# bacpop/sparrowhawk

Measured on AMD Instinct MI355X. Metric: Gbases/s assembled, k=31 150bp reads, higher is better.
Workload: dtype u64

## Files before the change

sparrowhawk_amd/csrc/ctl_words.h:

```cpp
#pragma once
#include <stddef.h>
#include <stdint.h>

namespace shk {

static constexpr int CTL_WORDS = 32;

struct CountWords {
    union { unsigned long long row_cursor;
            unsigned long long g_instances; };
    union { unsigned long long instances;
            unsigned long long g_overflow; };
    uint32_t part_too_large, bucket_splits;
    uint32_t n_handed_over, tally;
    unsigned long long bucket_list_len;
    unsigned long long spare5[4];
    unsigned long long bloom_keys;
    unsigned long long spare10;
    unsigned long long probe_work;
    unsigned long long dedupe_work;
    unsigned long long spare13;
    uint32_t groups_out, group_tally;
    unsigned long long spare15[7];
    unsigned long long er_cursor;
    unsigned long long er_broken;
    unsigned long long spare24[8];
};
struct P1Words {
    uint32_t spare, seg_too_long;
    unsigned long long max_fill;
};
struct CountMail {
    CountWords w;
    unsigned long long hist[500];
    P1Words p1;
};
static constexpr int COUNT_MAIL_WORDS = (int)(sizeof(CountMail) / 8);
static_assert(sizeof(CountMail) == (CTL_WORDS + 500 + 2) * 8 && offsetof(CountMail, hist) == CTL_WORDS * 8 && offsetof(CountMail, p1) == (CTL_WORDS + 500) * 8,
              "CountMail: words, histogram, pass 1's flags, contiguous");
static inline unsigned tally_tried(uint32_t t) { return t & 0xFFFFu; }
static inline unsigned tally_over(uint32_t t) { return t >> 16; }
static inline unsigned long long er_rows(unsigned long long cursor) { return cursor >> 32; }

struct GraphWords {
    unsigned long long spare0;
    unsigned long long table_flag;
    unsigned long long slots_used;
    unsigned long long n_cand, n_tips;
    union { unsigned long long tips_removed;
            unsigned long long n_splitters; };
    union { unsigned long long bubbles_removed;
            unsigned long long n_chains; };
    unsigned long long n_ring_splitters;
    uint32_t collapse_flag, n_spl_wanted;
    unsigned long long n_alive;
    unsigned long long n_walked;
    unsigned long long n_fork_cand;
    unsigned long long spare12;
    union { unsigned long long xq_count;
            unsigned long long halflink_flags; };
    unsigned long long writer_flag;
    unsigned long long spare15;
    unsigned long long r0_tips_removed, r0_bubbles_removed;
    unsigned long long plan_state, plan_bytes, plan_emitted;
    unsigned long long spare21[11];
};

#define SHK_CTL_AT(S, m, slot, half) static_assert(offsetof(S, m) == (slot) * 8 + (half) * 4, #S "::" #m " moved")
static_assert(sizeof(CountWords) == CTL_WORDS * 8 && sizeof(GraphWords) == CTL_WORDS * 8, "32 control words");
SHK_CTL_AT(CountWords, row_cursor, 0, 0);     SHK_CTL_AT(CountWords, g_instances, 0, 0);
SHK_CTL_AT(CountWords, instances, 1, 0);      SHK_CTL_AT(CountWords, g_overflow, 1, 0);
SHK_CTL_AT(CountWords, part_too_large, 2, 0); SHK_CTL_AT(CountWords, bucket_splits, 2, 1);
SHK_CTL_AT(CountWords, n_handed_over, 3, 0);  SHK_CTL_AT(CountWords, tally, 3, 1);
SHK_CTL_AT(CountWords, bucket_list_len, 4, 0);
SHK_CTL_AT(CountWords, bloom_keys, 9, 0);
SHK_CTL_AT(CountWords, probe_work, 11, 0);    SHK_CTL_AT(CountWords, dedupe_work, 12, 0);
SHK_CTL_AT(CountWords, groups_out, 14, 0);    SHK_CTL_AT(CountWords, group_tally, 14, 1);
SHK_CTL_AT(CountWords, er_cursor, 22, 0);     SHK_CTL_AT(CountWords, er_broken, 23, 0);
SHK_CTL_AT(GraphWords, spare0, 0, 0);         SHK_CTL_AT(GraphWords, table_flag, 1, 0);
SHK_CTL_AT(GraphWords, slots_used, 2, 0);     SHK_CTL_AT(GraphWords, n_cand, 3, 0);
SHK_CTL_AT(GraphWords, n_tips, 4, 0);
SHK_CTL_AT(GraphWords, tips_removed, 5, 0);   SHK_CTL_AT(GraphWords, n_splitters, 5, 0);
SHK_CTL_AT(GraphWords, bubbles_removed, 6, 0); SHK_CTL_AT(GraphWords, n_chains, 6, 0);
SHK_CTL_AT(GraphWords, n_ring_splitters, 7, 0);
SHK_CTL_AT(GraphWords, collapse_flag, 8, 0);  SHK_CTL_AT(GraphWords, n_spl_wanted, 8, 1);
SHK_CTL_AT(GraphWords, n_alive, 9, 0);        SHK_CTL_AT(GraphWords, n_walked, 10, 0);
SHK_CTL_AT(GraphWords, n_fork_cand, 11, 0);
SHK_CTL_AT(GraphWords, xq_count, 13, 0);      SHK_CTL_AT(GraphWords, halflink_flags, 13, 0);
SHK_CTL_AT(GraphWords, writer_flag, 14, 0);
SHK_CTL_AT(GraphWords, r0_tips_removed, 16, 0); SHK_CTL_AT(GraphWords, r0_bubbles_removed, 17, 0);
SHK_CTL_AT(GraphWords, plan_state, 18, 0);    SHK_CTL_AT(GraphWords, plan_bytes, 19, 0);
SHK_CTL_AT(GraphWords, plan_emitted, 20, 0);
#undef SHK_CTL_AT

}
```

sparrowhawk_amd/csrc/graph_part.h:

```cpp
#pragma once

struct MinScan {
    Nt32State first, last;
    uint32_t h_first, h_last;
    uint32_t min_wo_first;
    uint32_t min_wo_last;
    __device__ __forceinline__ uint32_t min_all() const { return min(min_wo_first, h_first); }
};

template <int W> __device__ __forceinline__ uint32_t km_base(const Kmer<W> &x, int k, int j) {
    return km_bits2<W>(x, 2 * (k - 1 - j));
}

template <int W> __device__ __forceinline__ MinScan km_min_scan(const Kmer<W> &x, int k, int gm) {
    MinScan r;
    Nt32State nt{0, 0};
    for (int j = 0; j < gm; j++) nt32_init_step(nt, km_base<W>(x, k, j), (unsigned)j);
    r.first = nt; r.h_first = nt32_canonical(nt);
    r.min_wo_first = 0xFFFFFFFFu; r.min_wo_last = r.h_first;
    const int w = k - gm + 1;
    uint32_t h = r.h_first;
    for (int q = 1; q < w; q++) {
        nt32_roll(nt, km_base<W>(x, k, q - 1), km_base<W>(x, k, q + gm - 1), (unsigned)gm);
        h = nt32_canonical(nt);
// ... 518 lines not shown
    const uint32_t *cnt;
    uint8_t *adj;
    GraphTable gt;
    const uint32_t *nb;
    int k;
    uint32_t n;
    uint32_t xref = 0;
    __device__ __forceinline__ uint32_t outmask(uint32_t v) const { return outmask_of(adj[v >> 1], v & 1); }
    __device__ __forceinline__ uint32_t outdeg(uint32_t v) const { return __popc(outmask(v)); }
    __device__ __forceinline__ uint32_t indeg(uint32_t v) const { return __popc(outmask(v ^ 1)); }
    __device__ __forceinline__ Kmer<W> seq(uint32_t v) const {
        Kmer<W> x = keys.load(v >> 1);
        return (v & 1) ? km_revcomp<W>(x, k) : x;
    }
    __device__ __forceinline__ uint32_t follow(uint32_t v, uint32_t b) const {
        Kmer<W> s = seq(v);
        km_push_back<W>(s, b, k);
        int o; Kmer<W> c = km_canonical<W>(s, k, o);
        uint32_t idx = gt_lookup<W>(gt, keys, c, k);
        return idx == NIL ? NIL : idx * 2 + (uint32_t)o;
    }
    __device__ __forceinline__ uint32_t only_out(uint32_t v) const {
        const uint32_t c = nb[v];
        if (c < NB_MULTI) return c;
        return follow(v, (uint32_t)__ffs((int)outmask(v)) - 1);
    }
};

struct TipRec { uint32_t start, junction, len, next; unsigned long long sum; };

template <int W>
__global__ __launch_bounds__(256) void k_tip_candidates(Graph<W> g, const uint8_t *__restrict__ alive,
                                                        uint32_t *__restrict__ cand,
                                                        unsigned int *__restrict__ n_cand,
                                                        uint2 *__restrict__ init_tip_head ,
                                                        uint8_t *__restrict__ init_mark ) {
    const int lane = threadIdx.x & 63;
    const uint32_t stride = gridDim.x * blockDim.x;
    const uint32_t n_round = (g.n + stride - 1) / stride * stride;
    for (uint32_t i = blockIdx.x * blockDim.x + threadIdx.x; i < n_round; i += stride) {
        uint32_t a = 0; bool al = false;
        if (i < g.n) {
            a = g.adj[i]; al = alive[i] != 0;
            if (init_tip_head) { uint2 nil; nil.x = NIL; nil.y = NIL; init_tip_head[i] = nil; init_mark[i] = 0; }
        }
#pragma unroll
        for (uint32_t o = 0; o < 2; o++) {
            const bool p = al && __popc(outmask_of(a, o ^ 1u)) == 0 && __popc(outmask_of(a, o)) == 1;
            const unsigned long long m = __ballot(p);
            if (!m) continue;
            unsigned int base = 0;
            if (lane == 0) base = atomicAdd(n_cand, (unsigned int)__popcll(m));
            base = __shfl(base, 0);
            if (p) cand[base + __popcll(m & ((1ull << lane) - 1ull))] = 2u * i + o;
        }
    }
}

template <int W>
__global__ __launch_bounds__(256) void k_tip_walk(Graph<W> g, const uint32_t *__restrict__ cand,
                                                  const unsigned int *__restrict__ n_cand_p, TipRec *__restrict__ tips,
                                                  unsigned int *__restrict__ n_tips,
                                                  uint32_t *__restrict__ tip_head) {
    const uint32_t T_TIP = 2u * (uint32_t)g.k;
    const uint32_t n_cand = *n_cand_p;
    for (uint32_t c = blockIdx.x * blockDim.x + threadIdx.x; c < n_cand; c += gridDim.x * blockDim.x) {
        const uint32_t v = cand[c];
        uint32_t cur = v, len = 1, J = NIL;
        unsigned long long sum = g.cnt[v >> 1];
        uint32_t a_cur = g.adj[cur >> 1], nb_cur = g.nb[cur];
        for (;;) {
            const uint32_t om = outmask_of(a_cur, cur & 1u);
            if (__popc(om) != 1) break;
            const uint32_t n = nb_cur < NB_MULTI ? nb_cur : g.follow(cur, (uint32_t)__ffs((int)om) - 1u);
            if (n == NIL) break;
            const uint32_t a_n = g.adj[n >> 1], nb_n = g.nb[n], c_n = g.cnt[n >> 1];
            if (__popc(outmask_of(a_n, (n & 1u) ^ 1u)) >= 2) { J = n; break; }
            len++; sum += c_n; cur = n; a_cur = a_n; nb_cur = nb_n;
            if (len > T_TIP) break;
        }
        if (J == NIL || len > T_TIP) continue;
        const uint32_t t = atomicAdd(n_tips, 1u);
        TipRec r; r.start = v; r.junction = J; r.len = len; r.sum = sum;
        r.next = atomicExch(&tip_head[J], t);
        tips[t] = r;
    }
}
// ... 42 lines not shown
}

__global__ __launch_bounds__(256) void k_tip_reset_heads(const TipRec *__restrict__ tips, const unsigned int *__restrict__ n_tips_p,
                                                         uint32_t *__restrict__ tip_head) {
    const uint32_t n_tips = *n_tips_p;
    for (uint32_t a = blockIdx.x * blockDim.x + threadIdx.x; a < n_tips; a += gridDim.x * blockDim.x)
        tip_head[tips[a].junction] = NIL;
}

template <int W>
__global__ __launch_bounds__(256) void k_fork_candidates(Graph<W> g, const uint8_t *__restrict__ alive,
                                                         uint32_t *__restrict__ cand,
                                                         unsigned int *__restrict__ n_cand) {
    const int lane = threadIdx.x & 63;
    const uint32_t stride = gridDim.x * blockDim.x;
    const uint32_t n_round = (g.n + stride - 1) / stride * stride;
    for (uint32_t i = blockIdx.x * blockDim.x + threadIdx.x; i < n_round; i += stride) {
        uint32_t a = 0; bool al = false;
        if (i < g.n) { a = g.adj[i]; al = alive[i] != 0; }
#pragma unroll
        for (uint32_t o = 0; o < 2; o++) {
            const bool p = al && __popc(outmask_of(a, o)) >= 2;
            const unsigned long long m = __ballot(p);
            if (!m) continue;
            unsigned int base = 0;
            if (lane == 0) base = atomicAdd(n_cand, (unsigned int)__popcll(m));
            base = __shfl(base, 0);
            if (p) cand[base + __popcll(m & ((1ull << lane) - 1ull))] = 2u * i + o;
        }
    }
}

template <int W>
__global__ __launch_bounds__(256) void k_bubble(Graph<W> g, const uint32_t *__restrict__ cand,
                                                const unsigned int *__restrict__ n_cand_p, uint8_t *__restrict__ mark) {
    const uint32_t T_BUB = 2u * (uint32_t)g.k;
    const uint32_t n_cand = *n_cand_p;
    for (uint32_t c = blockIdx.x * blockDim.x + threadIdx.x; c < n_cand; c += gridDim.x * blockDim.x) {
        const uint32_t S = cand[c];
        const uint32_t om = g.outmask(S);
        uint32_t first[4], end[4], len[4];
        unsigned long long sum[4];
        bool ok[4];
#pragma unroll
        for (uint32_t b = 0; b < 4; b++) {
            ok[b] = false; first[b] = NIL; end[b] = NIL; len[b] = 0; sum[b] = 0;
            if (!((om >> b) & 1u)) continue;
            const uint32_t bn = g.follow(S, b);
            if (bn == NIL || g.indeg(bn) != 1) continue;
            first[b] = bn;
            uint32_t cur = bn, l = 1;
            unsigned long long s = g.cnt[bn >> 1];
            for (;;) {
                if (g.outdeg(cur) != 1) break;
                const uint32_t n = g.only_out(cur);
                if (n == NIL) break;
                if (g.indeg(n) >= 2) { end[b] = n; ok[b] = true; break; }
                if (l + 1 > T_BUB) break;
                l++; s += g.cnt[n >> 1]; cur = n;
            }
            len[b] = l; sum[b] = s;
        }
#pragma unroll
        for (uint32_t a = 0; a < 4; a++) {
            if (!ok[a]) continue;
            const uint32_t E = end[a];
            {
                const Kmer<W> ks = g.keys.load(S >> 1), ke = g.keys.load(E >> 1);
                bool le;
                if (km_less<W>(ks, ke)) le = true;
                else if (km_less<W>(ke, ks)) le = false;
                else le = (S & 1u) <= ((E ^ 1u) & 1u);
                if (!le) continue;
            }
            uint32_t grp = 0; bool best = true;
            const Kmer<W> fa = g.keys.load(first[a] >> 1);
#pragma unroll
            for (uint32_t b = 0; b < 4; b++) {
                if (!ok[b] || end[b] != E) continue;
                grp++;
                if (b == a) continue;
                const unsigned long long l = sum[b] * len[a], r = sum[a] * len[b];
                bool better;
                if (l != r) better = l > r;
                else if (len[b] != len[a]) better = len[b] < len[a];
                else better = km_less<W>(g.keys.load(first[b] >> 1), fa);
                if (better) best = false;
            }
            if (grp >= 2 && !best) {
                uint32_t cur = first[a];
                for (uint32_t i = 0; i < len[a]; i++) {
                    mark[cur >> 1] = 1;
                    if (i + 1 < len[a]) cur = g.only_out(cur);
                }
            }
        }
    }
}

__global__ __launch_bounds__(256) void k_collect_marked(uint32_t n, uint8_t *__restrict__ mark,
                                                        uint8_t *__restrict__ alive,
                                                        uint32_t *__restrict__ removed,
                                                        unsigned int *__restrict__ n_removed) {
    const int lane = threadIdx.x & 63;
    const uint32_t stride = gridDim.x * blockDim.x;
    const uint32_t n_round = (n + stride - 1) / stride * stride;
    for (uint32_t i = blockIdx.x * blockDim.x + threadIdx.x; i < n_round; i += stride) {
        bool p = false;
        if (i < n && mark[i]) { mark[i] = 0; if (alive[i]) { alive[i] = 0; p = true; } }
        const unsigned long long m = __ballot(p);
        if (!m) continue;
        unsigned int base = 0;
        if (lane == 0) base = atomicAdd(n_removed, (unsigned int)__popcll(m));
        base = __shfl(base, 0);
        if (p) removed[base + __popcll(m & ((1ull << lane) - 1ull))] = i;
    }
}

__device__ __forceinline__ void adj_clear_bit(uint8_t *adj, uint32_t idx, uint32_t bit) {
    uint32_t *wptr = (uint32_t *)adj + (idx >> 2);
    atomicAnd(wptr, ~((1u << bit) << (8 * (idx & 3u))));
}

template <int W>
__global__ __launch_bounds__(256) void k_apply_removed(Graph<W> g, const uint32_t *__restrict__ removed,
                                                       const unsigned int *__restrict__ n_removed_p) {
    const uint32_t n_removed = *n_removed_p;
    for (uint32_t t = blockIdx.x * blockDim.x + threadIdx.x; t < n_removed; t += gridDim.x * blockDim.x) {
        const uint32_t r = removed[t];
        const uint32_t a = g.adj[r];
// ... 22 lines not shown
```

sparrowhawk_amd/csrc/pipeline.hip:

```cpp
#include <hip/hip_runtime.h>
#include <hipcub/hipcub.hpp>
#include <thread>
#include <stdint.h>
#include <stdio.h>
#include <stdlib.h>
#include <string.h>
#include <algorithm>
#include <atomic>
#include <chrono>
#include <map>
#include <memory>
#include <mutex>
#include <string>
#include <vector>

#include "ctl_words.h"
#include "device_mem.h"
#include "end_keys.h"
#include "kmer.h"
#include "pipeline.h"
#include "shard_comm.h"
#include "shard_plan.h"
#include "unitig_graph.h"
#include "unitig_graph_gpu.h"
// ... 1135 lines not shown
                            getenv("SHK_GP_ROWS") == nullptr && env_u64("SHK_GRAPH_RANGES", 1) != 0;
        er_ok_ = false;
        gp_ = 64;
        const uint64_t gp_rows_target = env_u64("SHK_GP_ROWS", 640);
        const uint64_t n_for_gp = sh_active_ ? n_solid_global_ : n;
        while (gp_ < GP_MAX && (uint64_t)gp_ * gp_rows_target < n_for_gp) gp_ <<= 1;
        if (ranges) gp_ = er_groups_;
        gt_slots_ = 4 * n + 8ull * gp_;
        if (int rc = gt_.alloc(gt_slots_, err)) return rc;
        if (int rc = gt_occ_.alloc(gt_slots_ / 8 + 8, err)) return rc;
        gt_scan_.release();
        if (!ranges && n && n <= (64ull << 20) && env_u64("SHK_KEEP_SCAN", 1)) if (int rc = gt_scan_.alloc(3 * n, err)) return rc;
        DevBuf<uint32_t> gp_of, gp_cnt, gp_roff, gp_rows, gp_n;
        if (ranges) {
            gt_off_.swap(er_off_); gt_msk_.swap(er_msk_); gp_roff.swap(er_start_); gp_n.swap(er_cnt_);
            er_off_.release(); er_msk_.release(); er_start_.release(); er_cnt_.release();
        } else {
            if (int rc = gt_off_.alloc(gp_, err)) return rc;
            if (int rc = gt_msk_.alloc(gp_, err)) return rc;
            if (int rc = gp_of.alloc(n, err)) return rc;
            if (int rc = gp_roff.alloc(gp_ + 1, err)) return rc;
            if (int rc = gp_rows.alloc(n, err)) return rc;
        }
        if (int rc = gp_cnt.alloc(gp_, err)) return rc;
        DevBuf<unsigned long long> queries;
        if (int rc = queries.alloc(8 * n + 8, err)) return rc;
        if (int rc = adj_.alloc((n + 8) & ~3ull, err)) return rc;
        if (keep_stages_) if (int rc = adj0_.alloc(n, err)) return rc;
        if (int rc = nb_.alloc(2 * n + 2, err)) return rc;
        if (int rc = alive_.alloc(n, err)) return rc;
        if (int rc = row_starts_.alloc(((n + 63) / 64) * 2 + 2, err)) return rc;
        if (ranges) HIPCHK(fill2_async(row_starts_.p, row_starts_.bytes, 0u, ctl_.p, sizeof(GraphWords), 0u, stream_));
        else HIPCHK(fill2_async(gp_cnt.p, (size_t)gp_ * 4, 0u, ctl_.p, sizeof(GraphWords), 0u, stream_));
        if (n || sh_active_) {
            Graph<W> g = graph_view();
            const uint32_t lowmask = std::min<uint32_t>(gp_, 256u) - 1u;
            if (ranges) {
                EvTimer t(stream_, stage_timers_);
                t.stop_later("graph_table_kernel", pending_timers_);
                EvTimer t2(stream_, stage_timers_);
                const GpRows gr{gp_roff.p, gp_n.p, nullptr};
                const uint32_t lds_slots = (uint32_t)std::min<uint64_t>(env_u64("SHK_GRAPH_LDS_SLOTS", ADJ_LDS_SLOTS_RANGES), ADJ_LDS_SLOTS_RANGES);
                hipLaunchKernelGGL((k_graph_local<W, ADJ_LDS_SLOTS_RANGES, ADJ_THREADS_RANGES>), dim3(gp_), dim3(ADJ_THREADS_RANGES), 0, stream_,
                                   g.keys, k_, g.gt, gr, adj_.p, nb_.p, queries.p, gp_cnt.p, (uint32_t *)ctl(&GraphWords::table_flag), lds_slots,
                                   alive_.p, row_starts_.p, lowmask);
                hipLaunchKernelGGL(k_graph_remote<W>, dim3(gp_), dim3(256), 0, stream_, g.keys, k_, g.gt, gr, queries.p,
                                   gp_cnt.p, adj_.p, nb_.p);
                HIPCHK(hipGetLastError());
                t2.stop_later("adjacency_kernel", pending_timers_);
                times_.add("graph_partitions_from_counting_x1", 1.0);
            } else {
                EvTimer t(stream_, stage_timers_);
                hipLaunchKernelGGL(k_gp_count<W>, dim3(grid_for(n)), dim3(256), 0, stream_, g.keys, (uint32_t)n, k_, g.gt,
                                   gp_of.p, gp_cnt.p);
                hipLaunchKernelGGL(k_gp_scan, dim3(1), dim3(1024), 0, stream_, gp_cnt.p, gp_, gt_off_.p, gt_msk_.p, gp_roff.p,
                                   ctl(&GraphWords::slots_used));
                hipLaunchKernelGGL(k_gp_rows, dim3(grid_for(n)), dim3(256), 0, stream_, gp_of.p, (uint32_t)n, gp_roff.p, gp_cnt.p,
                                   gp_rows.p);
                HIPCHK(hipGetLastError());
                if (n && (regroup_env == 1 || (regroup_env == 2 && rows_scattered_))) {
                    DevBuf<uint64_t> nk[W]; DevBuf<uint32_t> nc, ngp;
                    for (int j = 0; j < W; j++) if (int rc = nk[j].alloc(n, err)) return rc;
                    if (int rc = nc.alloc(n, err)) return rc;
                    if (int rc = ngp.alloc(n, err)) return rc;
                    KeyArr<W> out_keys; for (int j = 0; j < W; j++) out_keys.w[j] = nk[j].p;
                    hipLaunchKernelGGL(k_regroup_rows<W>, dim3(grid_for(n)), dim3(256), 0, stream_, g.keys, scnt_.p, gp_of.p, gp_rows.p, (uint32_t)n,
// ... 60 lines not shown
        unsigned long long h = 0;
        HIPCHK(hipMemcpyAsync(&h, ctl(m), ctl_span(m), hipMemcpyDeviceToHost, stream_));
        WAIT_STREAM();
        v = (unsigned int)h;
        return 0;
    }

    int apply_marks(Graph<W> &g, DevBuf<uint8_t> &mark, DevBuf<uint32_t> &removed, unsigned long long GraphWords::*m, std::string &err) {
        const uint32_t n = (uint32_t)n_solid_;
        hipLaunchKernelGGL(k_collect_marked, dim3(grid_for(n)), dim3(256), 0, stream_, n, mark.p, alive_.p,
                           removed.p, (unsigned int *)ctl(m));
        hipLaunchKernelGGL(k_apply_removed<W>, dim3(1024), dim3(256), 0, stream_, g, removed.p,
                           (const unsigned int *)ctl(m));
        HIPCHK(hipGetLastError());
        return 0;
    }

    int correct(bool tips, bool bubbles, std::string &err) override {
        if (!graph_ready_) { err = "graph not built"; return -2; }
        const uint32_t n = (uint32_t)n_solid_;
        tips_removed_ = bubbles_removed_ = 0; rounds_ = 0;
        corr_pending_ = false; corr_tips_ = tips; corr_bubbles_ = bubbles;
        if (n == 0 || (!tips && !bubbles)) return 0;
        if (int rc = corr_.cand.alloc(2ull * n, err)) return rc;
        if (int rc = corr_.removed.alloc(n, err)) return rc;
        if (int rc = corr_.mark.alloc(n, err)) return rc;
        if (!tips) HIPCHK(hipMemsetAsync(corr_.mark.p, 0, n, stream_));
        if (tips) {
            if (int rc = corr_.tip_head.alloc(2ull * n, err)) return rc;
            if (int rc = corr_.tiprec.alloc(2ull * n, err)) return rc;
            if (int rc = corr_.kill.alloc(2ull * n, err)) return rc;
        }
        EvTimer t(stream_, stage_timers_);
        if (int rc = correction_round(0, err)) return rc;
        t.stop_later("correct_total", pending_timers_);
        corr_pending_ = true;
        return 0;
    }
    struct CorrScratch { DevBuf<uint32_t> cand, tip_head, removed; DevBuf<uint8_t> mark, kill; DevBuf<TipRec> tiprec;
                         void release() { cand.release(); tip_head.release(); removed.release(); mark.release(); kill.release(); tiprec.release(); } };
    int correction_round(int round, std::string &err) {
        const uint32_t n = (uint32_t)n_solid_;
        Graph<W> g = graph_view();
        const dim3 G(1024), B(256);
        const bool tips = corr_tips_, bubbles = corr_bubbles_;
        const auto s_tip = round == 0 ? &GraphWords::r0_tips_removed : &GraphWords::tips_removed, s_bub = round == 0 ? &GraphWords::r0_bubbles_removed : &GraphWords::bubbles_removed;
        HIPCHK(fill_async(stream_, fill_region(ctl(&GraphWords::n_cand), ctl_span(&GraphWords::n_cand, &GraphWords::bubbles_removed), 0u),
                          fill_region(ctl(&GraphWords::n_fork_cand), ctl_span(&GraphWords::n_fork_cand), 0u)));
        unsigned int *const d_ncand = (unsigned int *)ctl(&GraphWords::n_cand), *const d_ntips = (unsigned int *)ctl(&GraphWords::n_tips);
        unsigned int *const d_nfork = (unsigned int *)ctl(&GraphWords::n_fork_cand);
        if (tips) {
            hipLaunchKernelGGL(k_tip_candidates<W>, dim3(grid_for(n)), B, 0, stream_, g, alive_.p,
                               corr_.cand.p, d_ncand, round == 0 ? (uint2 *)corr_.tip_head.p : (uint2 *)nullptr,
                               round == 0 ? corr_.mark.p : (uint8_t *)nullptr);
            hipLaunchKernelGGL(k_tip_walk<W>, G, B, 0, stream_, g, corr_.cand.p, (const unsigned int *)d_ncand,
                               corr_.tiprec.p, d_ntips, corr_.tip_head.p);
            hipLaunchKernelGGL(k_tip_decide<W>, G, B, 0, stream_, g, corr_.tiprec.p, (const unsigned int *)d_ntips,
                               corr_.tip_head.p, corr_.kill.p);
            hipLaunchKernelGGL(k_tip_remove<W>, G, B, 0, stream_, g, corr_.tiprec.p, (const unsigned int *)d_ntips,
                               corr_.kill.p, corr_.tip_head.p, corr_.mark.p);
            hipLaunchKernelGGL(k_tip_reset_heads, G, B, 0, stream_, corr_.tiprec.p, (const unsigned int *)d_ntips,
                               corr_.tip_head.p);
            HIPCHK(hipGetLastError());
            if (int rc = apply_marks(g, corr_.mark, corr_.removed, s_tip, err)) return rc;
        }
        if (bubbles) {
            hipLaunchKernelGGL(k_fork_candidates<W>, dim3(grid_for(n)), B, 0, stream_, g, alive_.p,
                               corr_.cand.p, d_nfork);
            hipLaunchKernelGGL(k_bubble<W>, G, B, 0, stream_, g, corr_.cand.p, (const unsigned int *)d_nfork, corr_.mark.p);
            HIPCHK(hipGetLastError());
            if (int rc = apply_marks(g, corr_.mark, corr_.removed, s_bub, err)) return rc;
        }
        return 0;
    }
    int finish_correction(unsigned int n1, unsigned int n2, std::string &err) {
        corr_pending_ = false;
        tips_removed_ += n1; bubbles_removed_ += n2; rounds_ = 1;
        EvTimer t(stream_, stage_timers_);
        for (int round = 1; round < 32 && n1 + n2 != 0; round++) {
            if (int rc = correction_round(round, err)) return rc;
            GraphWords *const h = (GraphWords *)(mbox64() + MB_MISC);
            HIPCHK(fetch_ctl(h, &GraphWords::tips_removed, &GraphWords::bubbles_removed));
            WAIT_STREAM();
            n1 = (unsigned int)h->tips_removed; n2 = (unsigned int)h->bubbles_removed;
            tips_removed_ += n1; bubbles_removed_ += n2; rounds_++;
        }
        if (rounds_ > 1) if (t.on()) times_.add("correct_total", t.stop());
        corr_.release();
        return 0;
    }

    int get_adjacency(uint8_t *adj_initial, uint8_t *adj_final, uint8_t *alive, uint64_t cap,
                      std::string &err) override {
        if (!graph_ready_) { err = "graph not built"; return -2; }
        if (cap < n_solid_) { err = "buffer too small"; return -1; }
        if (!n_solid_) return 0;
        if (adj_initial && !keep_stages_) { err = "the initial adjacency is kept for inspection only on a verbose handle (or with SHK_KEEP_STAGES=1)"; return -2; }
        if (adj_initial) HIPCHK(hipMemcpy(adj_initial, adj0_.p, n_solid_, hipMemcpyDeviceToHost));
        if (adj_final) HIPCHK(hipMemcpy(adj_final, adj_.p, n_solid_, hipMemcpyDeviceToHost));
        if (alive) HIPCHK(hipMemcpy(alive, alive_.p, n_solid_, hipMemcpyDeviceToHost));
        return 0;
    }

    struct ChainState {
        DevBuf<uint32_t> spl, slot_of;
        DevBuf<uint2> winfo, ol;
        DevBuf<SegRec> segs;
        DevBuf<FragRec> frag;
        DevBuf<RankRec> Ra, Rb;
        DevBuf<FinRec> fin;
        DevBuf<HeadRec> d_heads;
        DevBuf<RingMin> ringmin;
        std::vector<HeadRec> heads;
        uint32_t seg_cap = 0;
        unsigned int n_heads = 0;
        bool heads_on_host = true;
    };
    void stage_done(const char *who, unsigned id, const char *what) {
        const hipError_t e = hipStreamSynchronize(stream_);
        fprintf(stderr, "[%s%u] %s done%s\n", who, id, what, e == hipSuccess ? "" : " (stream error)");
// ... 3 lines not shown
    int rank_chains(ChainState &cs, bool rings, std::string &err, uint32_t keep_on_device_from = 0xFFFFFFFFu, EmitPlan *plan = nullptr) {
        const uint32_t n = (uint32_t)n_solid_;
        const uint32_t total = 2 * n;
        Graph<W> g = graph_view();
        if (plan) plan->planned = false;
        const bool stage_log = getenv("SHK_STAGE_LOG") != nullptr;
        auto stage = [&](const char *what) { if (stage_log) stage_done("rank_chains n=", n, what); };
        if (int rc = cs.winfo.alloc(total, err)) return rc;
        if (int rc = cs.frag.alloc(total, err)) return rc;
        if (int rc = cs.spl.alloc(total, err)) return rc;
        if (int rc = cs.ol.alloc(total, err)) return rc;
        const uint32_t split_mask = (1u << (uint32_t)env_u64("SHK_SPLIT_LOG", SPLIT_LOG_DEFAULT)) - 1u;
        const uint32_t tile_rows = (uint32_t)std::min<uint64_t>(std::max<uint64_t>(env_u64("SHK_TILE_ROWS", LF_ROWS), 1), LF_TILE / 2u);
        const int lf_grid = (int)((n + tile_rows - 1) / tile_rows);
        const uint64_t cap_all = std::min<uint64_t>((uint64_t)total + 1024u, 0xFFFFFFF0ull);
        uint64_t seg_cap64 = std::min<uint64_t>(cap_all, env_u64("SHK_SEG_CAP", (uint64_t)total / 12u + 65536u));
        constexpr unsigned int HEADS_SPEC = 512;
        static_assert(MB_MISC * 8 + HEADS_SPEC * sizeof(HeadRec) <= MBOX_BYTES, "mailbox");
        std::vector<HeadRec> &heads = cs.heads;
        GraphWords hc{};
        uint32_t seg_cap = 0;
        EvTimer tr(stream_, stage_timers_);
        for (int attempt = 0;; attempt++) {
            if (attempt > 3) { err = "collapse: the chain ranking did not settle"; return -6; }
            seg_cap = (uint32_t)seg_cap64;
            cs.seg_cap = seg_cap;
            if (int rc = cs.segs.alloc(seg_cap, err)) return rc;
            if (int rc = cs.Ra.alloc(seg_cap, err)) return rc;
            if (int rc = cs.Rb.alloc(seg_cap, err)) return rc;
            if (int rc = cs.slot_of.alloc(seg_cap, err)) return rc;
            if (int rc = cs.fin.alloc(seg_cap, err)) return rc;
            if (int rc = cs.d_heads.alloc(seg_cap, err)) return rc;
            if (int rc = cs.ringmin.alloc(seg_cap, err)) return rc;
            const unsigned long long *skip = corr_pending_ ? ctl(&GraphWords::r0_tips_removed) : (const unsigned long long *)nullptr;
            HIPCHK(fill_async(stream_, fill_region(ctl(&GraphWords::n_splitters), ctl_span(&GraphWords::n_splitters, &GraphWords::n_walked), 0u),
                              fill_region(ctl(&GraphWords::plan_state), ctl_span(&GraphWords::plan_state, &GraphWords::plan_emitted), 0u),
                              fill_region(cs.slot_of.p, (size_t)seg_cap * 4, 0xFFFFFFFFu)));
            unsigned int *d_nspl = (unsigned int *)ctl(&GraphWords::n_splitters), *d_nheads = (unsigned int *)ctl(&GraphWords::n_chains);
            uint32_t *d_flags = ctl(&GraphWords::collapse_flag);
            unsigned long long *d_plan = ctl(&GraphWords::plan_state);
            hipLaunchKernelGGL(k_succ_split<W>, dim3((total + 256 * SS_ITEMS - 1) / (256 * SS_ITEMS)), dim3(256), 0, stream_, g,
                               alive_.p, cs.winfo.p, cs.spl.p, cs.ol.p, d_nspl, split_mask, ctl(&GraphWords::n_alive), skip);
            stage("k_succ_split");
            hipLaunchKernelGGL(k_local_frag<W>, dim3(lf_grid), dim3(LF_THREADS), 0, stream_, n, row_starts_.p, tile_rows, alive_.p, cs.winfo.p, cs.ol.p, cs.frag.p, split_mask, skip,
                               d_nspl, seg_cap, d_flags);
            stage("k_local_frag");
            hipLaunchKernelGGL(k_walk_frags<W>, dim3(grid_for((uint64_t)total / 64u + 16384u, 256, 1 << 20)), dim3(256), 0, stream_,
                               cs.spl.p, (const unsigned int *)d_nspl, cs.frag.p, cs.segs.p, split_mask, ctl(&GraphWords::n_walked), total, d_flags);
            stage("k_walk_frags");
            hipLaunchKernelGGL(k_orphan_cycles<W>, dim3(grid_for(total)), dim3(256), 0, stream_, g, alive_.p, cs.winfo.p, cs.ol.p,
                               cs.frag.p, cs.spl.p, cs.segs.p, d_nspl, seg_cap, d_flags, ctl(&GraphWords::n_alive), ctl(&GraphWords::n_walked));
            HIPCHK(hipGetLastError());
            stage("k_orphan_cycles");
            const int gr = grid_for((uint64_t)total / 64u + 65536u);
            int rounds = 1; { uint64_t reach = RANK_HOPS; while (reach < (uint64_t)seg_cap + 1u) { reach *= RANK_HOPS; rounds++; } }
            hipLaunchKernelGGL(k_rank_init, dim3(gr), dim3(256), 0, stream_, cs.segs.p, (const unsigned int *)d_nspl, cs.Ra.p);
            RankRec *Ri = cs.Ra.p, *Ro = cs.Rb.p;
            for (int r = 0; r < rounds; r++) {
                hipLaunchKernelGGL(k_rank_jump, dim3(gr), dim3(256), 0, stream_, (const unsigned int *)d_nspl, Ri, Ro, (uint32_t)r);
                std::swap(Ri, Ro);
            }
            stage("k_rank_jump");
            unsigned int *d_ncyc = (unsigned int *)ctl(&GraphWords::n_ring_splitters);
            hipLaunchKernelGGL(k_rank_tails<W>, dim3(gr), dim3(256), 0, stream_, g, cs.segs.p, (const unsigned int *)d_nspl, Ri, cs.d_heads.p, cs.slot_of.p, cs.ringmin.p,
                               d_nheads, d_ncyc);
            hipLaunchKernelGGL(k_rank_fin, dim3(gr), dim3(256), 0, stream_, cs.segs.p, (const unsigned int *)d_nspl, Ri, cs.slot_of.p, cs.fin.p);
            stage("k_rank_tails + k_rank_fin");
            hipLaunchKernelGGL(k_tile_final, dim3(lf_grid), dim3(LF_THREADS), 0, stream_, n, row_starts_.p, tile_rows, cs.ol.p, cs.frag.p, cs.fin.p, skip, (const uint32_t *)d_flags);
            stage("k_tile_final");
            if (rings) {
                hipLaunchKernelGGL(k_ring_min1<W>, dim3(1024), dim3(256), 0, stream_, g, alive_.p, cs.ol.p, cs.ringmin.p, d_ncyc);
                hipLaunchKernelGGL(k_ring_min2<W>, dim3(1024), dim3(256), 0, stream_, g, alive_.p, cs.ol.p, cs.ringmin.p, d_ncyc);
                hipLaunchKernelGGL(k_ring_rot<W>, dim3(gr), dim3(256), 0, stream_, g, cs.d_heads.p, (const unsigned int *)d_nheads, cs.ringmin.p,
                                   cs.winfo.p, cs.ol.p, d_ncyc, d_flags);
            }
            if (plan) {
                hipLaunchKernelGGL(k_plan_emit, dim3(1), dim3(1024), 0, stream_, cs.d_heads.p, (const unsigned int *)d_nheads, (uint32_t)k_, plan->max_heads,
                                   plan->out_cap, (const uint32_t *)d_flags, plan->d_off, d_plan);
                hipLaunchKernelGGL(k_emit<W>, dim3(grid_for(n)), dim3(256), 0, stream_, g, alive_.p, cs.ol.p, plan->d_off, plan->d_out, (const unsigned long long *)d_plan);
            }
            HIPCHK(hipGetLastError());
            static_assert(sizeof(HeadRec) % 8 == 0, "chain records travel as 64-bit words");
            heads.assign(HEADS_SPEC, HeadRec());
            hipLaunchKernelGGL(k_mail_home, dim3(1), dim3(256), 0, stream_, (const unsigned long long *)ctl_.p, (uint32_t)CTL_WORDS, (const unsigned long long *)cs.d_heads.p,
                               (const unsigned int *)d_nheads, std::min<uint32_t>(HEADS_SPEC, seg_cap), (uint32_t)(sizeof(HeadRec) / 8), mbox64() + MB_CTL, mbox64() + MB_MISC);
            HIPCHK(hipGetLastError());
            if (plan) HIPCHK(hipMemcpyAsync(plan->h_out, plan->d_out, plan->out_cap, hipMemcpyDeviceToHost, stream_));
            WAIT_STREAM();
            const GraphWords &hc0 = *mb_graph();
            if (int rc = check_graph_flags(err)) return rc;
            if (corr_pending_) {
                const unsigned int r1 = (unsigned int)hc0.r0_tips_removed, r2 = (unsigned int)hc0.r0_bubbles_removed;
                if (int rc = finish_correction(r1, r2, err)) return rc;
                if (r1 + r2 != 0) continue;
            }
            hc = hc0;
            const uint32_t flag = hc.collapse_flag;
            if ((flag == 4 || flag == 2) && seg_cap64 < cap_all) {
                times_.add("collapse_seg_cap_retry_x1", 1.0);
                seg_cap64 = cap_all;
                continue;
            }
            memcpy(heads.data(), mbox64() + MB_MISC, (size_t)std::min<uint32_t>((uint32_t)std::min<unsigned long long>(hc.n_chains & 0xFFFFFFFFull, HEADS_SPEC), seg_cap) * sizeof(HeadRec));
            if (plan && hc.plan_state == 1ull) { plan->planned = true; plan->out_bytes = hc.plan_bytes; plan->n_emit = (uint32_t)hc.plan_emitted; }
            break;
        }
        if (hc.collapse_flag) { err = hc.collapse_flag == 2 ? "collapse: too many short circular unitigs" : (hc.collapse_flag == 3 ? "collapse: ring without a smallest k-mer" : "collapse: broken cycle"); return -6; }
        times_.add("collapse_n_splitters_x1e-3", (double)(unsigned int)hc.n_splitters * 1e-3);
        times_.add("collapse_cycle_splitters_x1e-3", (double)(unsigned int)hc.n_ring_splitters * 1e-3);
        const unsigned int n_heads = (unsigned int)hc.n_chains;
        if (tr.on()) times_.add("collapse_rank_device", tr.stop());
        cs.n_heads = n_heads;
        if (!rings || n_heads >= keep_on_device_from) { heads.resize(std::min<unsigned int>(n_heads, HEADS_SPEC)); cs.heads_on_host = false; return 0; }
        heads.resize(n_heads);
        cs.heads_on_host = true;
        if (n_heads > HEADS_SPEC)
            HIPCHK(hipMemcpy(heads.data() + HEADS_SPEC, cs.d_heads.p + HEADS_SPEC, (size_t)(n_heads - HEADS_SPEC) * sizeof(HeadRec), hipMemcpyDeviceToHost));
        return 0;
    }

    int collapse(std::vector<RawContig> &out, std::string &err, const char **json, size_t *json_len, uint64_t *n_contigs, TextArrival **arrival) override {
        out.clear();
        if (json) *json = nullptr;
        if (arrival) *arrival = nullptr;
        if (!graph_ready_) { err = "graph not built"; return -2; }
        const uint32_t n = (uint32_t)n_solid_;
        if (n == 0) return 0;
// ... 826 lines not shown
private:
    int k_;
    hipStream_t stream_ = nullptr; int stream_dev_ = 0;
    hipStream_t copy_stream_ = nullptr;
    ShardComm *wd_comm_ = nullptr;
    bool sh_agreed_ = false;
    StageTimes times_;
    std::vector<EvTimer::Pending> pending_timers_;
    int n_cus_ = 256;
    DevBuf<unsigned long long> ctl_;
    template <class S, class T> T *ctl(T S::*m) { return &(reinterpret_cast<S *>(ctl_.p)->*m); }
    template <class S, class A, class B> static size_t ctl_span(A S::*a, B S::*b) { static const S z{}; return (size_t)((const char *)&(z.*b) - (const char *)&(z.*a)) + sizeof(B); }
    template <class S, class A> static size_t ctl_span(A S::*a) { return sizeof(A); }
    template <class S, class A, class B> hipError_t fetch_ctl(S *img, A S::*a, B S::*b) { return hipMemcpyAsync(&(img->*a), ctl(a), ctl_span(a, b), hipMemcpyDeviceToHost, stream_); }
    PinnedBuf mbox_;
    unsigned long long *mbox64() { return (unsigned long long *)mbox_.p; }
    static constexpr size_t MBOX_BYTES = 32768;
    static constexpr int MB_COUNT = 0 , MB_CTL = COUNT_MAIL_WORDS , MB_MISC = MB_CTL + CTL_WORDS;
    CountMail *mb_count() { return (CountMail *)(mbox64() + MB_COUNT); }  GraphWords *mb_graph() { return (GraphWords *)(mbox64() + MB_CTL); }
    CountMail *d_count() { return reinterpret_cast<CountMail *>(ctl_.p); }
    hipError_t fetch_p1() { return hipMemcpyAsync(&mb_count()->p1, &d_count()->p1, sizeof(P1Words), hipMemcpyDeviceToHost, stream_); }
    hipError_t mail_count() {
        hipLaunchKernelGGL(k_mail_home, dim3(1), dim3(256), 0, stream_, (const unsigned long long *)ctl_.p, (uint32_t)COUNT_MAIL_WORDS, (const unsigned long long *)nullptr,
                           (const unsigned int *)nullptr, 0u, 0u, mbox64() + MB_COUNT, (unsigned long long *)nullptr);
        return hipGetLastError();
    }
    struct P1Pending { bool on; const uint32_t *d_bases, *d_seg_off; uint64_t n_seg, n_bases, cap; };
    P1Pending p1_{false, nullptr, nullptr, 0, 0, 0};
    bool p2_prefilled_ = false;
    uint64_t n_host_waits_ = 0;
    bool stage_timers_ = env_u64("SHK_STAGE_TIMERS", 0) != 0;
    bool keep_stages_ = env_u64("SHK_KEEP_STAGES", 0) != 0;
    bool graph_check_pending_ = false, corr_pending_ = false, corr_tips_ = false, corr_bubbles_ = false;
    CorrScratch corr_;
    bool defer_p1_ = false;
    uint64_t cap_override_ = 0;
    DevBuf<uint64_t> tkeys_[W]; DevBuf<uint32_t> tcnt_, tstate_; uint64_t tslots_ = 0;
    struct Batch { const uint32_t *bases, *seg_off; uint64_t n_seg; };
    std::vector<Batch> pending_;
    std::vector<DevPiece> piece_list_;
    uint64_t total_instances_ = 0, n_distinct_ = 0, n_solid_ = 0;
    uint64_t histo_[500] = {0};
    bool global_mode_ = env_u64("SHK_COUNT_MODE_GLOBAL", 0) != 0;
    bool bloom_ = false, bloom_off_once_ = false;
    bool have_parts_ = false;
    bool have_dedup_ = false;
    bool split_ready_ = false;
    std::vector<unsigned long long> split_base_; unsigned long long split_total_ = 0, split_stride_ = 0;
    DevBuf<uint64_t> dd_recs_; DevBuf<uint32_t> dd_w_, dd_n_; DevBuf<unsigned long long> dd_base_;
    PartParams pp_{};
    DevBuf<uint64_t> recs_; DevBuf<uint32_t> fill_;
    DevBuf<unsigned long long> run_off_; DevBuf<uint32_t> run_cnt_;
    RunView run_view_{}; uint32_t n_count_parts_ = 0; uint32_t forced_P_ = 0;
    std::vector<std::unique_ptr<BatchRecs>> batches_;
    const void *shard_recv_ = nullptr;
    DevBuf<uint64_t> ekeys_[W]; DevBuf<uint32_t> ecnt_;
    uint64_t n_emitted_ = 0; uint32_t emit_threshold_ = 0;
    bool rows_scattered_ = false;
    DevBuf<unsigned long long> er_off_; DevBuf<uint32_t> er_msk_, er_start_, er_cnt_;
    uint32_t er_groups_ = 0; uint64_t er_rows_ = 0; bool er_ok_ = false;
    DevBuf<uint64_t> skeys_[W]; DevBuf<uint32_t> scnt_;
    DevBuf<uint64_t> gt_; DevBuf<uint8_t> gt_occ_; DevBuf<uint2> gt_scan_; uint64_t gt_slots_ = 0; uint32_t gp_ = 64;
    DevBuf<unsigned long long> gt_off_; DevBuf<uint32_t> gt_msk_;
    DevBuf<uint8_t> adj_, adj0_, alive_;
    DevBuf<uint32_t> row_starts_;
    PinnedBuf hout_;
// ... 114 lines not shown
```

Measured before the change: 181.9.

## Speculate correction round zero: fused tip/fork candidates, defer removal until collapse check

Round zero of graph correction now runs a single fused candidate kernel that collects tip candidates from the front of the buffer and fork candidates from the back. It then walks tips and runs bubble detection speculatively, with bubble detection skipped once any tip exists. Tip/bubble removal and the apply_marks host syncs are deferred, so the speculative collapse proceeds and round zero is resumed only when tips or bubble marks were found. The aim is fewer kernel launches and host round-trips in the common clean-graph case. In exchange, control-word layout and round bookkeeping are more complex, and work may be redone when correction is needed.

New measurement: 180.8. About the same (-0.6%).

```diff
diff --git a/sparrowhawk_amd/csrc/ctl_words.h b/sparrowhawk_amd/csrc/ctl_words.h
--- a/sparrowhawk_amd/csrc/ctl_words.h
+++ b/sparrowhawk_amd/csrc/ctl_words.h
@@ -46,7 +46,7 @@
     unsigned long long spare0;
     unsigned long long table_flag;
     unsigned long long slots_used;
-    unsigned long long n_cand, n_tips;
+    unsigned long long n_cand, spare4;
     union { unsigned long long tips_removed;
             unsigned long long n_splitters; };
     union { unsigned long long bubbles_removed;
@@ -61,7 +61,7 @@
             unsigned long long halflink_flags; };
     unsigned long long writer_flag;
     unsigned long long spare15;
-    unsigned long long r0_tips_removed, r0_bubbles_removed;
+    unsigned long long n_tips, r0_marked;
     unsigned long long plan_state, plan_bytes, plan_emitted;
     unsigned long long spare21[11];
 };
@@ -79,7 +79,6 @@
 SHK_CTL_AT(CountWords, er_cursor, 22, 0);     SHK_CTL_AT(CountWords, er_broken, 23, 0);
 SHK_CTL_AT(GraphWords, spare0, 0, 0);         SHK_CTL_AT(GraphWords, table_flag, 1, 0);
 SHK_CTL_AT(GraphWords, slots_used, 2, 0);     SHK_CTL_AT(GraphWords, n_cand, 3, 0);
-SHK_CTL_AT(GraphWords, n_tips, 4, 0);
 SHK_CTL_AT(GraphWords, tips_removed, 5, 0);   SHK_CTL_AT(GraphWords, n_splitters, 5, 0);
 SHK_CTL_AT(GraphWords, bubbles_removed, 6, 0); SHK_CTL_AT(GraphWords, n_chains, 6, 0);
 SHK_CTL_AT(GraphWords, n_ring_splitters, 7, 0);
@@ -88,7 +87,7 @@
 SHK_CTL_AT(GraphWords, n_fork_cand, 11, 0);
 SHK_CTL_AT(GraphWords, xq_count, 13, 0);      SHK_CTL_AT(GraphWords, halflink_flags, 13, 0);
 SHK_CTL_AT(GraphWords, writer_flag, 14, 0);
-SHK_CTL_AT(GraphWords, r0_tips_removed, 16, 0); SHK_CTL_AT(GraphWords, r0_bubbles_removed, 17, 0);
+SHK_CTL_AT(GraphWords, n_tips, 16, 0);        SHK_CTL_AT(GraphWords, r0_marked, 17, 0);
 SHK_CTL_AT(GraphWords, plan_state, 18, 0);    SHK_CTL_AT(GraphWords, plan_bytes, 19, 0);
 SHK_CTL_AT(GraphWords, plan_emitted, 20, 0);
 #undef SHK_CTL_AT
diff --git a/sparrowhawk_amd/csrc/graph_part.h b/sparrowhawk_amd/csrc/graph_part.h
--- a/sparrowhawk_amd/csrc/graph_part.h
+++ b/sparrowhawk_amd/csrc/graph_part.h
@@ -574,18 +574,13 @@
 template <int W>
 __global__ __launch_bounds__(256) void k_tip_candidates(Graph<W> g, const uint8_t *__restrict__ alive,
                                                         uint32_t *__restrict__ cand,
-                                                        unsigned int *__restrict__ n_cand,
-                                                        uint2 *__restrict__ init_tip_head ,
-                                                        uint8_t *__restrict__ init_mark ) {
+                                                        unsigned int *__restrict__ n_cand) {
     const int lane = threadIdx.x & 63;
     const uint32_t stride = gridDim.x * blockDim.x;
     const uint32_t n_round = (g.n + stride - 1) / stride * stride;
     for (uint32_t i = blockIdx.x * blockDim.x + threadIdx.x; i < n_round; i += stride) {
         uint32_t a = 0; bool al = false;
-        if (i < g.n) {
-            a = g.adj[i]; al = alive[i] != 0;
-            if (init_tip_head) { uint2 nil; nil.x = NIL; nil.y = NIL; init_tip_head[i] = nil; init_mark[i] = 0; }
-        }
+        if (i < g.n) { a = g.adj[i]; al = alive[i] != 0; }
 #pragma unroll
         for (uint32_t o = 0; o < 2; o++) {
             const bool p = al && __popc(outmask_of(a, o ^ 1u)) == 0 && __popc(outmask_of(a, o)) == 1;
@@ -595,6 +590,41 @@
             if (lane == 0) base = atomicAdd(n_cand, (unsigned int)__popcll(m));
             base = __shfl(base, 0);
             if (p) cand[base + __popcll(m & ((1ull << lane) - 1ull))] = 2u * i + o;
+        }
+    }
+}
+
+template <int W>
+__global__ __launch_bounds__(256) void k_round0_candidates(Graph<W> g, const uint8_t *__restrict__ alive, uint32_t *__restrict__ cand,
+                                                           unsigned int *__restrict__ n_tip_cand, unsigned int *__restrict__ n_fork_cand,
+                                                           uint2 *__restrict__ init_tip_head, uint8_t *__restrict__ init_mark) {
+    const int lane = threadIdx.x & 63;
+    const uint32_t stride = gridDim.x * blockDim.x;
+    const uint32_t n_round = (g.n + stride - 1) / stride * stride;
+    const uint32_t last = 2u * g.n - 1u;
+    for (uint32_t i = blockIdx.x * blockDim.x + threadIdx.x; i < n_round; i += stride) {
+        uint32_t a = 0; bool al = false;
+        if (i < g.n) {
+            a = g.adj[i]; al = alive[i] != 0;
+            if (init_tip_head) { uint2 nil; nil.x = NIL; nil.y = NIL; init_tip_head[i] = nil; init_mark[i] = 0; }
+        }
+#pragma unroll
+        for (uint32_t o = 0; o < 2; o++) {
+            const uint32_t dout = __popc(outmask_of(a, o)), din = __popc(outmask_of(a, o ^ 1u));
+            const bool tip = n_tip_cand && al && din == 0 && dout == 1, fork = n_fork_cand && al && dout >= 2;
+            const unsigned long long mt = __ballot(tip), mf = __ballot(fork);
+            if (mt) {
+                unsigned int base = 0;
+                if (lane == 0) base = atomicAdd(n_tip_cand, (unsigned int)__popcll(mt));
+                base = __shfl(base, 0);
+                if (tip) cand[base + __popcll(mt & ((1ull << lane) - 1ull))] = 2u * i + o;
+            }
+            if (mf) {
+                unsigned int base = 0;
+                if (lane == 0) base = atomicAdd(n_fork_cand, (unsigned int)__popcll(mf));
+                base = __shfl(base, 0);
+                if (fork) cand[last - (base + __popcll(mf & ((1ull << lane) - 1ull)))] = 2u * i + o;
+            }
         }
     }
 }
@@ -703,12 +733,15 @@
 }
 
 template <int W>
-__global__ __launch_bounds__(256) void k_bubble(Graph<W> g, const uint32_t *__restrict__ cand,
-                                                const unsigned int *__restrict__ n_cand_p, uint8_t *__restrict__ mark) {
+__global__ __launch_bounds__(256) void k_bubble(Graph<W> g, const uint32_t *__restrict__ cand, int cand_dir,
+                                                const unsigned int *__restrict__ n_cand_p, uint8_t *__restrict__ mark,
+                                                const unsigned long long *__restrict__ stale, unsigned long long *__restrict__ n_marked) {
+    if (stale && *stale) return;
     const uint32_t T_BUB = 2u * (uint32_t)g.k;
     const uint32_t n_cand = *n_cand_p;
+    unsigned long long marked = 0;
     for (uint32_t c = blockIdx.x * blockDim.x + threadIdx.x; c < n_cand; c += gridDim.x * blockDim.x) {
-        const uint32_t S = cand[c];
+        const uint32_t S = cand[(long long)c * cand_dir];
         const uint32_t om = g.outmask(S);
         uint32_t first[4], end[4], len[4];
         unsigned long long sum[4];
@@ -764,9 +797,11 @@
                     mark[cur >> 1] = 1;
                     if (i + 1 < len[a]) cur = g.only_out(cur);
                 }
-            }
-        }
-    }
+                marked += len[a];
+            }
+        }
+    }
+    if (n_marked && marked) atomicAdd(n_marked, marked);
 }
 
 __global__ __launch_bounds__(256) void k_collect_marked(uint32_t n, uint8_t *__restrict__ mark,
diff --git a/sparrowhawk_amd/csrc/pipeline.hip b/sparrowhawk_amd/csrc/pipeline.hip
--- a/sparrowhawk_amd/csrc/pipeline.hip
+++ b/sparrowhawk_amd/csrc/pipeline.hip
@@ -1191,6 +1191,7 @@
         if (int rc = row_starts_.alloc(((n + 63) / 64) * 2 + 2, err)) return rc;
         if (ranges) HIPCHK(fill2_async(row_starts_.p, row_starts_.bytes, 0u, ctl_.p, sizeof(GraphWords), 0u, stream_));
         else HIPCHK(fill2_async(gp_cnt.p, (size_t)gp_ * 4, 0u, ctl_.p, sizeof(GraphWords), 0u, stream_));
+        corr_words_zero_ = true;
         if (n || sh_active_) {
             Graph<W> g = graph_view();
             const uint32_t lowmask = std::min<uint32_t>(gp_, 256u) - 1u;
@@ -1317,60 +1318,90 @@
             if (int rc = corr_.kill.alloc(2ull * n, err)) return rc;
         }
         EvTimer t(stream_, stage_timers_);
-        if (int rc = correction_round(0, err)) return rc;
+        Graph<W> g = graph_view();
+        if (!corr_words_zero_) HIPCHK(open_round_fill());
+        corr_words_zero_ = false;
+        unsigned int *const d_ncand = (unsigned int *)ctl(&GraphWords::n_cand), *const d_nfork = (unsigned int *)ctl(&GraphWords::n_fork_cand);
+        hipLaunchKernelGGL(k_round0_candidates<W>, dim3(grid_for(n)), dim3(256), 0, stream_, g, alive_.p, corr_.cand.p,
+                           tips ? d_ncand : (unsigned int *)nullptr, bubbles ? d_nfork : (unsigned int *)nullptr,
+                           tips ? (uint2 *)corr_.tip_head.p : (uint2 *)nullptr, tips ? corr_.mark.p : (uint8_t *)nullptr);
+        if (tips)
+            hipLaunchKernelGGL(k_tip_walk<W>, dim3(1024), dim3(256), 0, stream_, g, corr_.cand.p, (const unsigned int *)d_ncand,
+                               corr_.tiprec.p, (unsigned int *)ctl(&GraphWords::n_tips), corr_.tip_head.p);
+        if (bubbles)
+            hipLaunchKernelGGL(k_bubble<W>, dim3(1024), dim3(256), 0, stream_, g, corr_.cand.p + (2ull * n - 1), -1, (const unsigned int *)d_nfork,
+                               corr_.mark.p, (const unsigned long long *)ctl(&GraphWords::n_tips), ctl(&GraphWords::r0_marked));
+        HIPCHK(hipGetLastError());
         t.stop_later("correct_total", pending_timers_);
+        times_.add("correct_round0_speculative_x1", 1.0);
         corr_pending_ = true;
         return 0;
     }
     struct CorrScratch { DevBuf<uint32_t> cand, tip_head, removed; DevBuf<uint8_t> mark, kill; DevBuf<TipRec> tiprec;
                          void release() { cand.release(); tip_head.release(); removed.release(); mark.release(); kill.release(); tiprec.release(); } };
-    int correction_round(int round, std::string &err) {
-        const uint32_t n = (uint32_t)n_solid_;
+    hipError_t open_round_fill() {
+        return fill_async(stream_, fill_region(ctl(&GraphWords::n_cand), ctl_span(&GraphWords::n_cand, &GraphWords::bubbles_removed), 0u),
+                          fill_region(ctl(&GraphWords::n_fork_cand), ctl_span(&GraphWords::n_fork_cand), 0u),
+                          fill_region(ctl(&GraphWords::n_tips), ctl_span(&GraphWords::n_tips, &GraphWords::r0_marked), 0u));
+    }
+    int remove_tips(Graph<W> &g, std::string &err) {
+        const dim3 G(1024), B(256);
+        const unsigned int *const d_ntips = (const unsigned int *)ctl(&GraphWords::n_tips);
+        hipLaunchKernelGGL(k_tip_decide<W>, G, B, 0, stream_, g, corr_.tiprec.p, d_ntips, corr_.tip_head.p, corr_.kill.p);
+        hipLaunchKernelGGL(k_tip_remove<W>, G, B, 0, stream_, g, corr_.tiprec.p, d_ntips, corr_.kill.p, corr_.tip_head.p, corr_.mark.p);
+        hipLaunchKernelGGL(k_tip_reset_heads, G, B, 0, stream_, corr_.tiprec.p, d_ntips, corr_.tip_head.p);
+        HIPCHK(hipGetLastError());
+        return apply_marks(g, corr_.mark, corr_.removed, &GraphWords::tips_removed, err);
+    }
+    int remove_bubbles(Graph<W> &g, std::string &err) {
+        unsigned int *const d_nfork = (unsigned int *)ctl(&GraphWords::n_fork_cand);
+        hipLaunchKernelGGL(k_fork_candidates<W>, dim3(grid_for(g.n)), dim3(256), 0, stream_, g, alive_.p, corr_.cand.p, d_nfork);
+        hipLaunchKernelGGL(k_bubble<W>, dim3(1024), dim3(256), 0, stream_, g, corr_.cand.p, 1, (const unsigned int *)d_nfork, corr_.mark.p,
+                           (const unsigned long long *)nullptr, (unsigned long long *)nullptr);
+        HIPCHK(hipGetLastError());
+        return apply_marks(g, corr_.mark, corr_.removed, &GraphWords::bubbles_removed, err);
+    }
+    int correction_round(std::string &err) {
         Graph<W> g = graph_view();
-        const dim3 G(1024), B(256);
-        const bool tips = corr_tips_, bubbles = corr_bubbles_;
-        const auto s_tip = round == 0 ? &GraphWords::r0_tips_removed : &GraphWords::tips_removed, s_bub = round == 0 ? &GraphWords::r0_bubbles_removed : &GraphWords::bubbles_removed;
-        HIPCHK(fill_async(stream_, fill_region(ctl(&GraphWords::n_cand), ctl_span(&GraphWords::n_cand, &GraphWords::bubbles_removed), 0u),
+        HIPCHK(open_round_fill());
+        if (corr_tips_) {
+            unsigned int *const d_ncand = (unsigned int *)ctl(&GraphWords::n_cand);
+            hipLaunchKernelGGL(k_tip_candidates<W>, dim3(grid_for(g.n)), dim3(256), 0, stream_, g, alive_.p, corr_.cand.p, d_ncand);
+            hipLaunchKernelGGL(k_tip_walk<W>, dim3(1024), dim3(256), 0, stream_, g, corr_.cand.p, (const unsigned int *)d_ncand,
+                               corr_.tiprec.p, (unsigned int *)ctl(&GraphWords::n_tips), corr_.tip_head.p);
+            if (int rc = remove_tips(g, err)) return rc;
+        }
+        if (corr_bubbles_) if (int rc = remove_bubbles(g, err)) return rc;
+        return 0;
+    }
+    int continue_round0(unsigned int n_tips, std::string &err) {
+        Graph<W> g = graph_view();
+        HIPCHK(fill_async(stream_, fill_region(ctl(&GraphWords::tips_removed), ctl_span(&GraphWords::tips_removed, &GraphWords::bubbles_removed), 0u),
                           fill_region(ctl(&GraphWords::n_fork_cand), ctl_span(&GraphWords::n_fork_cand), 0u)));
-        unsigned int *const d_ncand = (unsigned int *)ctl(&GraphWords::n_cand), *const d_ntips = (unsigned int *)ctl(&GraphWords::n_tips);
-        unsigned int *const d_nfork = (unsigned int *)ctl(&GraphWords::n_fork_cand);
-        if (tips) {
-            hipLaunchKernelGGL(k_tip_candidates<W>, dim3(grid_for(n)), B, 0, stream_, g, alive_.p,
-                               corr_.cand.p, d_ncand, round == 0 ? (uint2 *)corr_.tip_head.p : (uint2 *)nullptr,
-                               round == 0 ? corr_.mark.p : (uint8_t *)nullptr);
-            hipLaunchKernelGGL(k_tip_walk<W>, G, B, 0, stream_, g, corr_.cand.p, (const unsigned int *)d_ncand,
-                               corr_.tiprec.p, d_ntips, corr_.tip_head.p);
-            hipLaunchKernelGGL(k_tip_decide<W>, G, B, 0, stream_, g, corr_.tiprec.p, (const unsigned int *)d_ntips,
-                               corr_.tip_head.p, corr_.kill.p);
-            hipLaunchKernelGGL(k_tip_remove<W>, G, B, 0, stream_, g, corr_.tiprec.p, (const unsigned int *)d_ntips,
-                               corr_.kill.p, corr_.tip_head.p, corr_.mark.p);
-            hipLaunchKernelGGL(k_tip_reset_heads, G, B, 0, stream_, corr_.tiprec.p, (const unsigned int *)d_ntips,
-                               corr_.tip_head.p);
-            HIPCHK(hipGetLastError());
-            if (int rc = apply_marks(g, corr_.mark, corr_.removed, s_tip, err)) return rc;
-        }
-        if (bubbles) {
-            hipLaunchKernelGGL(k_fork_candidates<W>, dim3(grid_for(n)), B, 0, stream_, g, alive_.p,
-                               corr_.cand.p, d_nfork);
-            hipLaunchKernelGGL(k_bubble<W>, G, B, 0, stream_, g, corr_.cand.p, (const unsigned int *)d_nfork, corr_.mark.p);
-            HIPCHK(hipGetLastError());
-            if (int rc = apply_marks(g, corr_.mark, corr_.removed, s_bub, err)) return rc;
-        }
-        return 0;
-    }
-    int finish_correction(unsigned int n1, unsigned int n2, std::string &err) {
+        if (n_tips) {
+            if (int rc = remove_tips(g, err)) return rc;
+            if (corr_bubbles_) if (int rc = remove_bubbles(g, err)) return rc;
+        } else if (int rc = apply_marks(g, corr_.mark, corr_.removed, &GraphWords::bubbles_removed, err)) return rc;
+        times_.add("correct_round0_continued_x1", 1.0);
+        return 0;
+    }
+    int finish_correction(unsigned int n_tips, unsigned long long n_marked, std::string &err) {
         corr_pending_ = false;
-        tips_removed_ += n1; bubbles_removed_ += n2; rounds_ = 1;
+        rounds_ = 0;
         EvTimer t(stream_, stage_timers_);
-        for (int round = 1; round < 32 && n1 + n2 != 0; round++) {
-            if (int rc = correction_round(round, err)) return rc;
+        const bool resumed = n_tips != 0 || n_marked != 0;
+        bool more = resumed;
+        for (int round = 0; round < 32 && more; round++) {
+            if (int rc = round == 0 ? continue_round0(n_tips, err) : correction_round(err)) return rc;
             GraphWords *const h = (GraphWords *)(mbox64() + MB_MISC);
             HIPCHK(fetch_ctl(h, &GraphWords::tips_removed, &GraphWords::bubbles_removed));
             WAIT_STREAM();
-            n1 = (unsigned int)h->tips_removed; n2 = (unsigned int)h->bubbles_removed;
+            const unsigned int n1 = (unsigned int)h->tips_removed, n2 = (unsigned int)h->bubbles_removed;
             tips_removed_ += n1; bubbles_removed_ += n2; rounds_++;
-        }
-        if (rounds_ > 1) if (t.on()) times_.add("correct_total", t.stop());
+            more = n1 + n2 != 0;
+        }
+        if (!resumed) rounds_ = 1;
+        if (resumed) if (t.on()) times_.add("correct_total", t.stop());
         corr_.release();
         return 0;
     }
@@ -1440,7 +1471,7 @@
             if (int rc = cs.fin.alloc(seg_cap, err)) return rc;
             if (int rc = cs.d_heads.alloc(seg_cap, err)) return rc;
             if (int rc = cs.ringmin.alloc(seg_cap, err)) return rc;
-            const unsigned long long *skip = corr_pending_ ? ctl(&GraphWords::r0_tips_removed) : (const unsigned long long *)nullptr;
+            const unsigned long long *skip = corr_pending_ ? ctl(&GraphWords::n_tips) : (const unsigned long long *)nullptr;
             HIPCHK(fill_async(stream_, fill_region(ctl(&GraphWords::n_splitters), ctl_span(&GraphWords::n_splitters, &GraphWords::n_walked), 0u),
                               fill_region(ctl(&GraphWords::plan_state), ctl_span(&GraphWords::plan_state, &GraphWords::plan_emitted), 0u),
                               fill_region(cs.slot_of.p, (size_t)seg_cap * 4, 0xFFFFFFFFu)));
@@ -1498,9 +1529,9 @@
             const GraphWords &hc0 = *mb_graph();
             if (int rc = check_graph_flags(err)) return rc;
             if (corr_pending_) {
-                const unsigned int r1 = (unsigned int)hc0.r0_tips_removed, r2 = (unsigned int)hc0.r0_bubbles_removed;
-                if (int rc = finish_correction(r1, r2, err)) return rc;
-                if (r1 + r2 != 0) continue;
+                const unsigned int r0_tips = (unsigned int)hc0.n_tips; const unsigned long long r0_marked = hc0.r0_marked;
+                if (int rc = finish_correction(r0_tips, r0_marked, err)) return rc;
+                if (r0_tips != 0 || r0_marked != 0) continue;
             }
             hc = hc0;
             const uint32_t flag = hc.collapse_flag;
@@ -2393,6 +2424,7 @@
     bool stage_timers_ = env_u64("SHK_STAGE_TIMERS", 0) != 0;
     bool keep_stages_ = env_u64("SHK_KEEP_STAGES", 0) != 0;
     bool graph_check_pending_ = false, corr_pending_ = false, corr_tips_ = false, corr_bubbles_ = false;
+    bool corr_words_zero_ = false;
     CorrScratch corr_;
     bool defer_p1_ = false;
     uint64_t cap_override_ = 0;
```
